# getterupper/PreWorld

Measured on AMD Instinct MI355X. Metric: samples/sec (6-cam frame -> 200x200x16 occ), higher is better.
Workload: dtype f32 as hi+lo f16 (3 MFMA per product block, f32 accumulate)

## Files before the change

### preworld_amd/csrc/pw_conv3d_common.h

```cpp
#ifndef PW_CONV3D_COMMON_H_
#define PW_CONV3D_COMMON_H_
#include "pw_common.h"

#include <stdlib.h>

typedef float f32x16 __attribute__((ext_vector_type(16)));

namespace {
constexpr int BD = 4, BH = 8, BW = 8;
constexpr int TD = BD + 2, TH = BH + 2, TW = BW + 2;
constexpr int TV = TD * TH * TW;
constexpr unsigned WPIECE = 1024u;
constexpr int KC = 32;
}

struct ConvArgs {
  const float* x;
  const float* wpk;
  const float* scale;
  const float* bias;
  const float* residual;
  float* y0;
  float* y1;
  int B, D, H, W, Cin;
// ... 111 lines not shown
  for (int mt = 0; mt < 2; ++mt) {
#pragma unroll
    for (int q = 0; q < 4; ++q) {
      const float av[4] = {aq[mt][q].x, aq[mt][q].y, aq[mt][q].z, aq[mt][q].w};
#pragma unroll
      for (int e = 0; e < 4; ++e) {
#pragma unroll
        for (int nt = 0; nt < NT; ++nt) {
          const float bv[4] = {b[nt][q].x, b[nt][q].y, b[nt][q].z, b[nt][q].w};
          acc[mt][nt] = __builtin_amdgcn_mfma_f32_32x32x2f32(av[e], bv[e], acc[mt][nt], 0, 0, 0);
        }
      }
    }
  }
}

template <int NT, int TAP>
__device__ __forceinline__ void tap_pair(const float* lds, const unsigned (&aaddr)[2][3][4],
                                         rsrc_t wr, unsigned wsoff, unsigned lane_off, unsigned wstride,
                                         float4 (&b0)[NT][4], float4 (&b1)[NT][4],
                                         f32x16 (&acc)[2][NT]) {
  if constexpr (TAP + 1 < 27) {
    load_b<NT>(wr, wsoff + (unsigned)(TAP + 1) * wstride, lane_off, b1);
    __builtin_amdgcn_sched_barrier(0);
    tap_mfma<NT, TAP>(lds, aaddr, b0, acc);
    __builtin_amdgcn_sched_barrier(0);
    load_b<NT>(wr, wsoff + (unsigned)(TAP + 2) * wstride, lane_off, b0);
    __builtin_amdgcn_sched_barrier(0);
    tap_mfma<NT, TAP + 1>(lds, aaddr, b1, acc);
    __builtin_amdgcn_sched_barrier(0);
    tap_pair<NT, TAP + 2>(lds, aaddr, wr, wsoff, lane_off, wstride, b0, b1, acc);
  } else {
    tap_mfma<NT, TAP>(lds, aaddr, b0, acc);
  }
}

__device__ __forceinline__ constexpr int acc_patch(int r, int h) {
  const int i = (r & 3) + 8 * (r >> 2) + 4 * h;
  const int g = i >> 2;
  const int set = (0x96 >> g) & 1;
  return set * 16 + (g >> 1) * 4 + (i & 3);
}

__device__ __forceinline__ int xcd_contiguous(int bid, int nblk) {
  const int x = bid & 7, idx = bid >> 3;
  const int q = nblk >> 3, r = nblk & 7;
  return x * q + min(x, r) + idx;
}

typedef __attribute__((address_space(3))) char* lds3_t;
constexpr unsigned PIPE_OOB = 0xfffffff0u;
constexpr int PIPE_BUF_BYTES = TV * KC * 4;
constexpr int PIPE_ROWS_PER_WAVE = TD * TH / 4;

struct PipeDma {
  unsigned voff[2][2];
  int b, d0, h0, wbase, ch;
  unsigned ldsbuf;
  bool live;
};

__device__ __forceinline__ void pipe_lane_offsets(const ConvArgs& a, int w0, int lane, unsigned (&voff)[2][2]) {
  const int shift = w0 == 0 ? 1 : 0;
  {
    const int ww = lane >> 3, slot = lane & 7;
    const bool wok = (unsigned)(w0 - 1 + ww) < (unsigned)a.W;
#pragma unroll
    for (int par = 0; par < 2; ++par) {
      const int f = ((ww >> 1) & 3) | (par << 2);
      voff[par][0] = wok ? (unsigned)((ww - shift) * a.Cin + (slot ^ f) * 4) * 4u : PIPE_OOB;
    }
  }
  {
    const int ww = 8 + (lane >> 5), dw = lane & 31, slot = dw >> 2;
    const bool wok = (unsigned)(w0 - 1 + ww) < (unsigned)a.W;
#pragma unroll
    for (int par = 0; par < 2; ++par) {
      const int f = ((ww >> 1) & 3) | (par << 2);
      voff[par][1] = wok ? (unsigned)((ww - shift) * a.Cin + (slot ^ f) * 4 + (dw & 3)) * 4u : PIPE_OOB;
    }
  }
}

template <int K>
__device__ __forceinline__ void pipe_dma_row(const ConvArgs& a, rsrc_t xr, lds3_t lds3, const PipeDma& dm,
                                             int wave) {
  const int row = wave + 4 * K;
  const int dd = row / TH, hh = row - dd * TH;
  const int gd = dm.d0 + dd - 1, gh = dm.h0 + hh - 1;
  const bool rok = dm.live && (unsigned)gd < (unsigned)a.D && (unsigned)gh < (unsigned)a.H;
  const unsigned soff = rok ? (unsigned)(((((dm.b * a.D + gd) * a.H + gh) * a.W + dm.wbase) * a.Cin + dm.ch * KC) * 4) : 0u;
  const unsigned v0 = rok ? ((hh & 1) ? dm.voff[1][0] : dm.voff[0][0]) : PIPE_OOB;
  const unsigned v1 = rok ? ((hh & 1) ? dm.voff[1][1] : dm.voff[0][1]) : PIPE_OOB;
  lds3_t dst = lds3 + (dm.ldsbuf + (unsigned)row * (TW * 128));
  __builtin_amdgcn_raw_ptr_buffer_load_lds(xr, dst, 16, v0, soff, 0, 0);
  __builtin_amdgcn_raw_ptr_buffer_load_lds(xr, dst + 1024, 4, v1, soff, 0, 0);
}


__device__ __forceinline__ void stage_halo_chunk_dma(const ConvArgs& a, rsrc_t xr, float* lds, int b, int d0,
                                                     int h0, int w0, int ch, int wave, int lane) {
  if (ch > 0) __syncthreads();
  PipeDma dm;
  pipe_lane_offsets(a, w0, lane, dm.voff);
  dm.b = b; dm.d0 = d0; dm.h0 = h0; dm.wbase = w0 > 0 ? w0 - 1 : 0; dm.ch = ch; dm.ldsbuf = 0; dm.live = true;
  const lds3_t lds3 = (lds3_t)lds;
  pipe_dma_row<0>(a, xr, lds3, dm, wave); pipe_dma_row<1>(a, xr, lds3, dm, wave); pipe_dma_row<2>(a, xr, lds3, dm, wave);
  pipe_dma_row<3>(a, xr, lds3, dm, wave); pipe_dma_row<4>(a, xr, lds3, dm, wave); pipe_dma_row<5>(a, xr, lds3, dm, wave);
  pipe_dma_row<6>(a, xr, lds3, dm, wave); pipe_dma_row<7>(a, xr, lds3, dm, wave); pipe_dma_row<8>(a, xr, lds3, dm, wave);
  pipe_dma_row<9>(a, xr, lds3, dm, wave); pipe_dma_row<10>(a, xr, lds3, dm, wave); pipe_dma_row<11>(a, xr, lds3, dm, wave);
  pipe_dma_row<12>(a, xr, lds3, dm, wave); pipe_dma_row<13>(a, xr, lds3, dm, wave); pipe_dma_row<14>(a, xr, lds3, dm, wave);
  __builtin_amdgcn_s_waitcnt(0);
  __syncthreads();
}


struct PipeArgs {
  unsigned m_ng, m_tw, m_th, m_td;
  int ngroups, n_items;
};


__device__ __forceinline__ int udiv_magic(int x, int d, unsigned magic) {
  return d == 1 ? x : (int)__umulhi((unsigned)x, magic);
}

struct PipeTile { int b, d0, h0, w0, ng; };

__device__ __forceinline__ PipeTile pipe_decode(const ConvArgs& a, const PipeArgs& p, int item) {
  PipeTile t;
  int tile = udiv_magic(item, p.ngroups, p.m_ng);
  t.ng = item - tile * p.ngroups;
  int q = udiv_magic(tile, a.tiles_w, p.m_tw);
  t.w0 = (tile - q * a.tiles_w) * BW; tile = q;
  q = udiv_magic(tile, a.tiles_h, p.m_th);
  t.h0 = (tile - q * a.tiles_h) * BH; tile = q;
  q = udiv_magic(tile, a.tiles_d, p.m_td);
  t.d0 = (tile - q * a.tiles_d) * BD;
  t.b = q;
  return t;
}


template <typename K>
static int set_lds_limit(K kernel, int bytes) {
  PW_CHECK_HIP(hipFuncSetAttribute(reinterpret_cast<const void*>(kernel),
                                   hipFuncAttributeMaxDynamicSharedMemorySize, bytes));
  return PW_OK;
}

static inline unsigned magic_of(int d) { return d <= 1 ? 0u : (unsigned)((1ull << 32) / (unsigned)d) + 1u; }

static inline int pw_num_cus() {
  static int n = 0;
  if (!n) {
    int dev = 0;
    hipDeviceProp_t pr;
    if (hipGetDevice(&dev) == hipSuccess && hipGetDeviceProperties(&pr, dev) == hipSuccess) n = pr.multiProcessorCount;
    if (n < 8) n = 256;
  }
  return n;
}

static inline bool use_pipe(long long n_items, int NT, int algo) {
  if (algo == 1 || algo == 4) return algo == 4 && n_items < (1ll << 20);
  return NT == 1 && n_items >= 512 && n_items < (1ll << 20);
}

int pw_launch_conv3d_gather(const ConvArgs& a, int NT, int ngroups, int ksize, int stride, int algo, int Cin,
                             long long n_out, hipStream_t st, bool f16 = false);
int pw_launch_conv3d_h2_s2(const ConvArgs& a, hipStream_t st);

#endif
```

### preworld_amd/csrc/pw_conv3d_h2.hip

```cpp
#include "pw_h2.h"

namespace {
constexpr int H2_SB_OFF = 2 * PIPE_BUF_BYTES;
constexpr int H2_MAX_COUT = 256;
constexpr int H2_LDS = H2_SB_OFF + 2 * H2_MAX_COUT * 4;
}

struct EpiTile { int b, d0, h0, w0, ng; unsigned bufoff; bool pending; };
struct EpiRegs {
  v4f x0, x1, s0, s1, b0, b1; float4 r0, r1; unsigned vbase, soff;
  float amax0, amax1;
  float amax_nt[2];
};

template <int NT>
__device__ __forceinline__ void epi_fold_amax(const ConvArgs& a, int ng, EpiRegs& r) {
#pragma unroll
  for (int nt = 0; nt < NT; ++nt) {
    const bool to_y0 = (ng * NT + nt) * 32 < a.cout0;
    r.amax0 = fmaxf(r.amax0, to_y0 ? r.amax_nt[nt] : 0.f);
    r.amax1 = fmaxf(r.amax1, to_y0 ? 0.f : r.amax_nt[nt]);
    r.amax_nt[nt] = 0.f;
  }
}

__device__ __forceinline__ unsigned epi_slot_off(int u) {
  const int row = (int)(((unsigned)u * 205u) >> 11);
  return (unsigned)(row * (4 * TW * 128) + (u - row * 10) * 128);
}

template <int NT>
__device__ __forceinline__ void h2_epi_park(const f32x16 (&acc)[2][NT], char* stg, int lane) {
  const int half = lane >> 5, pj = patch_of_row(lane & 31);
#pragma unroll
  for (int nt = 0; nt < NT; ++nt)
#pragma unroll
    for (int mt = 0; mt < 2; ++mt) {
      const int u = nt * 64 + mt * 32 + pj;
      char* dst = stg + epi_slot_off(u);
      const int sw = (u >> 1) & 7;
#pragma unroll
      for (int g = 0; g < 4; ++g) {
        v4f v;
#pragma unroll
        for (int e = 0; e < 4; ++e) v[e] = acc[mt][nt][4 * g + e];
        *reinterpret_cast<v4f*>(dst + (((2 * g + half) ^ sw) * 16)) = v;
      }
    }
}

template <int NT, int EPI, int P>
__device__ __forceinline__ void h2_epi_load(const ConvArgs& a, const EpiTile& t, const char* stg, const float* sb, int wave,
                                            int lane, EpiRegs& r) {
  constexpr int nt = P >> 2;
  const int n0 = (t.ng * NT + nt) * 32;
  const bool to_y0 = n0 < a.cout0;
  const int ld = to_y0 ? a.ld0 : a.ld1;
  const int col0 = to_y0 ? n0 : n0 - a.n1_start;
  const int od = t.d0 + wave;
  const int o = lane & 3;
  const int u = 16 * P + (lane >> 2), sv = u & 63;
  const int mt = sv >> 5, vr = (sv >> 3) & 3, vc = sv & 7;
  const bool ok = (int)t.pending & (int)(od < a.Do) & (int)((t.h0 + mt * 4 + vr) < a.Ho) & (int)((t.w0 + vc) < a.Wo);
  r.soff = (unsigned)(((((t.b * a.Do + od) * a.Ho + t.h0) * a.Wo + t.w0) * ld) * 4);
  const unsigned pos = (EPI == 3 ? (unsigned)(32 * o) : (unsigned)((4 * (o & 1) + 2 * (o >> 1)) * 16));
  const unsigned vin = (unsigned)(((mt * 4 + vr) * a.Wo + vc) * ld) * 4u + (unsigned)col0 * 4u + pos;
  r.vbase = ok ? vin : PIPE_OOB;
  const char* src = stg + epi_slot_off(u);
  const int sw = (u >> 1) & 7;
  r.x0 = *reinterpret_cast<const v4f*>(src + (((2 * o) ^ sw) * 16));
  r.x1 = *reinterpret_cast<const v4f*>(src + (((2 * o + 1) ^ sw) * 16));
  r.s0 = *reinterpret_cast<const v4f*>(sb + n0 + 8 * o);
  r.s1 = *reinterpret_cast<const v4f*>(sb + n0 + 8 * o + 4);
  r.b0 = *reinterpret_cast<const v4f*>(sb + H2_MAX_COUT + n0 + 8 * o);
  r.b1 = *reinterpret_cast<const v4f*>(sb + H2_MAX_COUT + n0 + 8 * o + 4);
  if constexpr (EPI == 2) {
    const unsigned out_vox = (unsigned)((size_t)a.B * a.Do * a.Ho * a.Wo);
    const rsrc_t rr = make_rsrc(a.residual, out_vox * (unsigned)ld * 4u);
    r.r0 = buf_load4(rr, r.vbase, r.soff);
    r.r1 = buf_load4(rr, r.vbase == PIPE_OOB ? PIPE_OOB : r.vbase + 16u, r.soff);
  }
}

template <int NT, int EPI, int P>
__device__ __forceinline__ void h2_epi_compute(const ConvArgs& a, const EpiTile& t, EpiRegs& r, float res_mul) {
  constexpr int nt = P >> 2;
  const int n0 = (t.ng * NT + nt) * 32;
  const bool to_y0 = n0 < a.cout0;
  float* dst = to_y0 ? a.y0 : a.y1;
  const int ld = to_y0 ? a.ld0 : a.ld1;
  const float lo_clamp = (to_y0 ? a.relu0 : a.relu1) ? 0.f : -3.402823466e38f;
  const unsigned out_vox = (unsigned)((size_t)a.B * a.Do * a.Ho * a.Wo);
  const rsrc_t yr = make_rsrc(dst, out_vox * (unsigned)ld * 4u);
  float v[8];
#pragma unroll
  for (int e = 0; e < 4; ++e) { v[e] = fmaf(r.x0[e], r.s0[e], r.b0[e]); v[4 + e] = fmaf(r.x1[e], r.s1[e], r.b1[e]); }
  if constexpr (EPI == 2) {
    const h8 rh = __builtin_bit_cast(h8, r.r0), rl = __builtin_bit_cast(h8, r.r1);
#pragma unroll
    for (int e = 0; e < 8; ++e) v[e] = fmaf((float)rh[e] + (float)rl[e], res_mul, v[e]);
  }
#pragma unroll
  for (int e = 0; e < 8; ++e) v[e] = fmaxf(v[e], lo_clamp);
  {
    float m = fabsf(v[0]);
#pragma unroll
    for (int e = 1; e < 8; ++e) m = fmaxf(m, fabsf(v[e]));
    r.amax_nt[nt] = fmaxf(r.amax_nt[nt], r.vbase == PIPE_OOB ? 0.f : m);
  }
  const unsigned second = r.vbase == PIPE_OOB ? PIPE_OOB : r.vbase + 16u;
  if constexpr (EPI == 3) {
    const float va[4] = {v[0], v[1], v[2], v[3]}, vb[4] = {v[4], v[5], v[6], v[7]};
    buf_store4(yr, r.vbase, r.soff, va);
    buf_store4(yr, second, r.soff, vb);
  } else {
    h8 oh, ol;
    h2_split8(v, oh, ol);
    const v4f wh = __builtin_bit_cast(v4f, oh), wl = __builtin_bit_cast(v4f, ol);
    const float va[4] = {wh[0], wh[1], wh[2], wh[3]}, vb[4] = {wl[0], wl[1], wl[2], wl[3]};
    buf_store4(yr, r.vbase, r.soff, va);
    buf_store4(yr, second, r.soff, vb);
  }
}

template <int NT, int EPI, int P>
__device__ __forceinline__ void h2_epi_rest(const ConvArgs& a, const EpiTile& t, const char* stg, const float* sb, int wave,
                                            int lane, EpiRegs& r, float res_mul) {
  if constexpr (P < 4 * NT) {
    h2_epi_load<NT, EPI, P>(a, t, stg, sb, wave, lane, r);
    h2_epi_compute<NT, EPI, P>(a, t, r, res_mul);
    h2_epi_rest<NT, EPI, P + 1>(a, t, stg, sb, wave, lane, r, res_mul);
  }
}

#ifndef PW_DMA_ROWS_PER_TAP_NT1
#define PW_DMA_ROWS_PER_TAP_NT1 3
#endif
#ifndef PW_DMA_ROWS_PER_TAP_NT2
#define PW_DMA_ROWS_PER_TAP_NT2 5
#endif
template <int NT, int TAP>
__device__ __forceinline__ constexpr int h2_dma_first_row() {
  constexpr int per = NT == 1 ? PW_DMA_ROWS_PER_TAP_NT1 : PW_DMA_ROWS_PER_TAP_NT2, t0 = 4 * NT + 2;
  return TAP < t0 ? PIPE_ROWS_PER_WAVE : (TAP - t0) * per;
}
template <int NT, int TAP>
__device__ __forceinline__ constexpr int h2_dma_row_count() {
  constexpr int per = NT == 1 ? PW_DMA_ROWS_PER_TAP_NT1 : PW_DMA_ROWS_PER_TAP_NT2;
  constexpr int k0 = h2_dma_first_row<NT, TAP>();
  return k0 >= PIPE_ROWS_PER_WAVE ? 0 : (k0 + per <= PIPE_ROWS_PER_WAVE ? per : PIPE_ROWS_PER_WAVE - k0);
}

template <int NT>
struct H2Ctx {
  lds3_t lds3;
  rsrc_t xr, wr;
  unsigned lane_off, wstride;
  unsigned wsoff, wsoff_next;
  bool has_next;
  PipeDma dm;
  unsigned dm_base, dm_pitch;
  int wave, lane;
  long long* tap_probe;
  EpiTile epi;
  const char* ldsg;
  float res_mul;
};

template <int TAP>
__device__ __forceinline__ void h2_read_a_tap(lds3_t lds3, const unsigned (&aaddr)[2][3][4], v4f (&aq)[2][4]) {
  constexpr int kd = TAP / 9, kh = (TAP / 3) % 3, kw = TAP % 3;
#pragma unroll
  for (int mt = 0; mt < 2; ++mt) {
    constexpr unsigned imm0 = (unsigned)(((kd * TH + kh) * TW) * 128);
    const unsigned imm = imm0 + (unsigned)(mt * 4 * TW * 128);
#pragma unroll
    for (int q = 0; q < 4; ++q)
      aq[mt][q] = *reinterpret_cast<const __attribute__((address_space(3))) v4f*>(lds3 + aaddr[kh & 1][kw][q] + imm);
  }
}

template <int NT, bool WR = false>
__device__ __forceinline__ void h2_load_b(rsrc_t wr, unsigned wsoff, unsigned lane_off, v4f (&b)[NT][4]) {
#pragma unroll
  for (int nt = 0; nt < NT; ++nt)
#pragma unroll
    for (int q = WR ? 1 : 0; q < 4; q += WR ? 2 : 1) {
      const auto v = __builtin_amdgcn_raw_buffer_load_b128(wr, lane_off + (unsigned)q * H2W_PIECE, wsoff + (unsigned)(nt * 4096), 0);
      v4f o;
      o[0] = __uint_as_float(v[0]); o[1] = __uint_as_float(v[1]); o[2] = __uint_as_float(v[2]); o[3] = __uint_as_float(v[3]);
      b[nt][q] = o;
    }
}

template <int NT, bool WR = false, int TAP = 0, int NW = 1>
__device__ __forceinline__ void h2_mfma(const v4f (&aq)[2][4], const v4f (&b)[NT][4], f32x16 (&acc)[2][NT], const v4f (&wres)[NW][2]) {
#pragma unroll
  for (int ks = 0; ks < 2; ++ks) {
#pragma unroll
    for (int prod = 0; prod < 3; ++prod) {
      const int pw = prod == 1 ? 1 : 0, px = prod == 2 ? 1 : 0;
#pragma unroll
      for (int mt = 0; mt < 2; ++mt)
#pragma unroll
        for (int nt = 0; nt < NT; ++nt) {
          v4f w = b[nt][2 * ks + pw];
          if constexpr (WR) { if (pw == 0) w = wres[TAP][ks]; }
          acc[mt][nt] = __builtin_amdgcn_mfma_f32_32x32x16_f16(__builtin_bit_cast(h8, w), __builtin_bit_cast(h8, aq[mt][2 * ks + px]),
                                                               acc[mt][nt], 0, 0, 0);
        }
    }
  }
}
template <int NT>
__device__ __forceinline__ void h2_mfma(const v4f (&aq)[2][4], const v4f (&b)[NT][4], f32x16 (&acc)[2][NT]) {
  const v4f none[1][2] = {};
  h2_mfma<NT, false, 0, 1>(aq, b, acc, none);
}

__device__ __forceinline__ constexpr int h2_share(int i, int slots, int n) { return ((i + 1) * n) / slots - (i * n) / slots; }

template <int I, int S, int NVM, int NDS, int NSA, int NVA>
__device__ __forceinline__ void h2_pipeline() {
  if constexpr (I < S) {
    __builtin_amdgcn_sched_group_barrier(0x008, 1, 0);
    if constexpr (h2_share(I, S, NDS) > 0) __builtin_amdgcn_sched_group_barrier(0x100, h2_share(I, S, NDS), 0);
    if constexpr (h2_share(I, S, NVM) > 0) __builtin_amdgcn_sched_group_barrier(0x020, h2_share(I, S, NVM), 0);
    if constexpr (h2_share(I, S, NSA) > 0) __builtin_amdgcn_sched_group_barrier(0x004, h2_share(I, S, NSA), 0);
    if constexpr (h2_share(I, S, NVA) > 0) __builtin_amdgcn_sched_group_barrier(0x002, h2_share(I, S, NVA), 0);
    h2_pipeline<I + 1, S, NVM, NDS, NSA, NVA>();
  }
}

struct H2DmaView { rsrc_t xr; lds3_t lds3; unsigned base, pitch; int wave; };
template <int K>
__device__ __forceinline__ void h2_dma_row(const ConvArgs& a, const PipeDma& dm, const H2DmaView& c) {
  constexpr int c1 = (4 * K) / TH, c2 = (4 * K) % TH;
  const int t = c2 + c.wave;
  const int carry = t >= TH ? 1 : 0;
  const int dd = c1 + carry, hh = t - TH * carry;
  const bool rok = (int)dm.live & (int)((unsigned)(dm.d0 - 1 + dd) < (unsigned)a.D) & (int)((unsigned)(dm.h0 - 1 + hh) < (unsigned)a.H);
  const unsigned soff = c.base + (unsigned)(dd * a.H + hh) * c.pitch;
#ifdef PW_X_DMAOOB
  const unsigned v0 = rok ? PIPE_OOB : PIPE_OOB - 16u, v1 = v0;
#else
  const unsigned v0 = rok ? ((hh & 1) ? dm.voff[1][0] : dm.voff[0][0]) : PIPE_OOB;
  const unsigned v1 = rok ? ((hh & 1) ? dm.voff[1][1] : dm.voff[0][1]) : PIPE_OOB;
#endif
  lds3_t dst = c.lds3 + (dm.ldsbuf + (unsigned)(c1 * TH + c2) * (TW * 128) + (unsigned)c.wave * (TW * 128));
  __builtin_amdgcn_raw_ptr_buffer_load_lds(c.xr, dst, 16, v0, soff, 0, 0);
  __builtin_amdgcn_raw_ptr_buffer_load_lds(c.xr, dst + 1024, 4, v1, soff, 0, 0);
}

template <int K0, int N>
__device__ __forceinline__ void h2_dma_rows(const ConvArgs& a, const PipeDma& dm, const H2DmaView& c) {
  if constexpr (N > 0) {
    h2_dma_row<K0>(a, dm, c);
    h2_dma_rows<K0 + 1, N - 1>(a, dm, c);
  }
}

template <int NT, int EPI, int TAP, bool WR = false, int NW = 1>
__device__ __forceinline__ void h2_step(const ConvArgs& a, const H2Ctx<NT>& c, const unsigned (&aaddr)[2][3][4],
                                        v4f (&ac)[2][4], v4f (&an)[2][4], v4f (&b0)[NT][4], v4f (&b1)[NT][4],
                                        v4f (&b2)[NT][4], f32x16 (&acc)[2][NT], EpiRegs& er, const v4f (&wres)[NW][2]) {
#ifdef PW_CONV_TAP_PROBE
  if (c.tap_probe) {
    if (c.lane == 0) c.tap_probe[c.wave * 27 + TAP] = __builtin_readcyclecounter();
  }
#endif
  __builtin_amdgcn_sched_barrier(0);
  constexpr int dma_k0 = h2_dma_first_row<NT, TAP>(), dma_n = h2_dma_row_count<NT, TAP>();
#ifdef PW_X_NOEPI
  constexpr bool epi_tap = false, epi_ld = false;
#else
  constexpr bool epi_tap = EPI > 0 && TAP >= 2 && TAP <= 4 * NT + 1;
  constexpr bool epi_ld = EPI > 0 && TAP >= 1 && TAP <= 4 * NT;
#endif
#ifdef PW_X_BSAME
  h2_load_b<NT, WR>(c.wr, c.wsoff, c.lane_off, b2);
#elif !defined(PW_X_NOB)
  if constexpr (TAP + 2 < 27) {
    h2_load_b<NT, WR>(c.wr, c.wsoff + (unsigned)(TAP + 2) * c.wstride, c.lane_off, b2);
  } else {
    h2_load_b<NT, WR>(c.wr, c.wsoff_next + (unsigned)(TAP + 2 - 27) * c.wstride, c.lane_off, b2);
  }
#endif
#ifndef PW_X_NODMA
  h2_dma_rows<dma_k0, dma_n>(a, c.dm, H2DmaView{c.xr, c.lds3, c.dm_base, c.dm_pitch, c.wave});
#endif
#ifndef PW_X_NOA
  if constexpr (TAP < 26) h2_read_a_tap<TAP + 1>(c.lds3, aaddr, an);
#endif
  if constexpr (epi_tap) h2_epi_compute<NT, EPI, TAP - 2>(a, c.epi, er, c.res_mul);
  if constexpr (epi_ld)
    h2_epi_load<NT, EPI, TAP - 1>(a, c.epi, c.ldsg + c.epi.bufoff + (unsigned)c.wave * (TW * 128),
                                  reinterpret_cast<const float*>(c.ldsg + H2_SB_OFF), c.wave, c.lane, er);
  h2_mfma<NT, WR, TAP, NW>(ac, b0, acc, wres);
  {
    constexpr int n_vm = (WR ? 2 : 4) * NT + 2 * dma_n + ((epi_ld && EPI == 2) ? 2 : 0);
    constexpr int n_ds = (TAP < 26 ? 8 : 0) + (epi_ld ? 6 : 0);
    constexpr int n_sa = 4 + 26 * dma_n + (epi_ld ? 12 : 0);
    constexpr int n_va = 5 * dma_n + (epi_tap ? (EPI == 2 ? 100 : 76) : 0) + (epi_ld ? 36 : 0);
    h2_pipeline<0, 12 * NT, n_vm, n_ds, n_sa, n_va>();
    if constexpr (epi_tap) __builtin_amdgcn_sched_group_barrier(0x040, 2, 0);
  }
  __builtin_amdgcn_sched_barrier(0);
  if constexpr (TAP < 26) h2_step<NT, EPI, TAP + 1, WR, NW>(a, c, aaddr, an, ac, b1, b2, b0, acc, er, wres);
}

template <int NT>
__device__ __forceinline__ void h2_epilogue(const ConvArgs& a, const f32x16 (&acc)[2][NT], const float* sb, char* stg,
                                            int b, int d0, int h0, int w0, int ng, int wave, int lane, float res_mul,
                                            float& amax0, float& amax1) {
  const int od = d0 + wave;
  const int half = lane >> 5, pj = patch_of_row(lane & 31);
  const unsigned out_vox = (unsigned)((size_t)a.B * a.Do * a.Ho * a.Wo);
  constexpr unsigned STG_ROW = 4 * TW * 128;
#pragma unroll
  for (int nt = 0; nt < NT; ++nt) {
    const int n0 = (ng * NT + nt) * 32;
    const bool to_y0 = n0 < a.cout0;
    float* dst = to_y0 ? a.y0 : a.y1;
    if (dst == nullptr) continue;
    const int stride = to_y0 ? a.cout0 : a.cout1;
    const int ld = to_y0 ? a.ld0 : a.ld1;
    const int col0 = to_y0 ? n0 : n0 - a.n1_start;
    if (col0 < 0 || col0 >= stride) continue;
    const int fmt = to_y0 ? a.fmt_y0 : a.fmt_y1;
    const float lo_clamp = (to_y0 ? a.relu0 : a.relu1) ? 0.f : -3.402823466e38f;
    const bool has_res = to_y0 && a.residual != nullptr;
    const rsrc_t yr = make_rsrc(dst, out_vox * (unsigned)ld * 4u);
    const rsrc_t rr = make_rsrc(has_res ? a.residual : dst, out_vox * (unsigned)ld * 4u);
#pragma unroll
    for (int g = 0; g < 4; ++g) {
      const v4f sc = *reinterpret_cast<const v4f*>(sb + n0 + 8 * g + 4 * half);
      const v4f bi = *reinterpret_cast<const v4f*>(sb + H2_MAX_COUT + n0 + 8 * g + 4 * half);
#pragma unroll
      for (int mt = 0; mt < 2; ++mt) {
        const int sv = mt * 32 + pj;
        v4f v;
#pragma unroll
        for (int e = 0; e < 4; ++e) v[e] = fmaf(acc[mt][nt][4 * g + e], sc[e], bi[e]);
        *reinterpret_cast<v4f*>(stg + (sv >> 3) * STG_ROW + (sv & 7) * 128 + (((2 * g + half) ^ ((sv >> 1) & 7)) * 16)) = v;
      }
    }
    const int o = lane & 3;
#pragma unroll
    for (int q = 0; q < 4; ++q) {
      const int sv = 16 * q + (lane >> 2);
      const int mt = sv >> 5, vr = (sv >> 3) & 3, vc = sv & 7;
      const bool ok = od < a.Do && (h0 + mt * 4 + vr) < a.Ho && (w0 + vc) < a.Wo;
      const unsigned soff = (unsigned)(((((b * a.Do + od) * a.Ho + h0) * a.Wo + w0) * ld) * 4);
      const unsigned vox = (unsigned)(((mt * 4 + vr) * a.Wo + vc) * ld) * 4u + (unsigned)col0 * 4u;
      const char* src = stg + (sv >> 3) * STG_ROW + (sv & 7) * 128;
      const int sw = (sv >> 1) & 7;
      const v4f lo4 = *reinterpret_cast<const v4f*>(src + (((2 * o) ^ sw) * 16));
      const v4f hi4 = *reinterpret_cast<const v4f*>(src + (((2 * o + 1) ^ sw) * 16));
      float v[8] = {lo4[0], lo4[1], lo4[2], lo4[3], hi4[0], hi4[1], hi4[2], hi4[3]};
      const unsigned pos = (fmt == 0 ? (unsigned)(32 * o) : (unsigned)((4 * (o & 1) + 2 * (o >> 1)) * 16));
      const unsigned rpos = (a.fmt_res == 0 ? (unsigned)(32 * o) : (unsigned)((4 * (o & 1) + 2 * (o >> 1)) * 16));
      if (has_res) {
        const unsigned base = ok ? vox + rpos : PIPE_OOB;
        const float4 r0 = buf_load4(rr, base, soff), r1 = buf_load4(rr, ok ? base + 16u : PIPE_OOB, soff);
        if (a.fmt_res == 0) {
          const float rv[8] = {r0.x, r0.y, r0.z, r0.w, r1.x, r1.y, r1.z, r1.w};
#pragma unroll
          for (int e = 0; e < 8; ++e) v[e] = fmaf(rv[e], res_mul, v[e]);
        } else {
          const h8 rh = __builtin_bit_cast(h8, r0), rl = __builtin_bit_cast(h8, r1);
#pragma unroll
          for (int e = 0; e < 8; ++e) v[e] = fmaf((float)rh[e] + (float)rl[e], res_mul, v[e]);
        }
      }
#pragma unroll
      for (int e = 0; e < 8; ++e) v[e] = fmaxf(v[e], lo_clamp);
      if (ok) {
        float m = fabsf(v[0]);
#pragma unroll
        for (int e = 1; e < 8; ++e) m = fmaxf(m, fabsf(v[e]));
        if (to_y0) amax0 = fmaxf(amax0, m); else amax1 = fmaxf(amax1, m);
      }
      const unsigned obase = ok ? vox + pos : PIPE_OOB;
      if (fmt == 0) {
        const float va[4] = {v[0], v[1], v[2], v[3]}, vb[4] = {v[4], v[5], v[6], v[7]};
        buf_store4(yr, obase, soff, va);
        buf_store4(yr, ok ? obase + 16u : PIPE_OOB, soff, vb);
      } else {
        h8 oh, ol;
        h2_split8(v, oh, ol);
        const v4f wh = __builtin_bit_cast(v4f, oh), wl = __builtin_bit_cast(v4f, ol);
        const float va[4] = {wh[0], wh[1], wh[2], wh[3]}, vb[4] = {wl[0], wl[1], wl[2], wl[3]};
        buf_store4(yr, obase, soff, va);
        buf_store4(yr, ok ? obase + 16u : PIPE_OOB, soff, vb);
      }
    }
  }
}

template <int NT, int EPI, bool WR = false>
__global__ void __launch_bounds__(256, 1) k_conv3d_h2(ConvArgs a, PipeArgs p) {
#ifdef PW_X_SKIP_SMALLCONV
  if ((long long)a.D * a.H * a.W <= 80000) return;
#endif
#ifdef PW_X_SKIP_BIGCONV
  if ((long long)a.D * a.H * a.W > 80000) return;
#endif
  extern __shared__ __attribute__((aligned(16))) float lds[];
  const int tid = threadIdx.x, lane = tid & 63;
  const int wave = uni(tid >> 6);
  const int half = lane >> 5, j = lane & 31;
  const int pj = patch_of_row(j), pr = pj >> 3, pc = pj & 7;
  const int ntiles_total = a.cout_total >> 5;
  const int nchunk = a.Cin / KC;

  const RngScale rs = rng_scales(a);

  const int nslots = (int)gridDim.x >> 3;
  const int per = (p.n_items + 7) >> 3;
  const int it_end = min(((int)blockIdx.x & 7) * per + per, p.n_items);
  int item = ((int)blockIdx.x & 7) * per + ((int)blockIdx.x >> 3);
  if (item >= it_end) return;

  unsigned aaddr0[2][3][4];
#pragma unroll
  for (int khp = 0; khp < 2; ++khp)
#pragma unroll
    for (int kw = 0; kw < 3; ++kw) {
      const int ww = pc + kw;
      const int f = ((ww >> 1) & 3) | (((pr + khp) & 1) << 2);
#pragma unroll
      for (int q = 0; q < 4; ++q)
        aaddr0[khp][kw][q] = (unsigned)((((wave * TH + pr) * TW + ww) * 8 + ((half * 4 + q) ^ f)) * 16);
    }

  H2Ctx<NT> c;
  c.lds3 = (lds3_t)lds;
  c.xr = make_rsrc(a.x, (unsigned)((size_t)a.B * a.D * a.H * a.W * a.Cin * 4));
  c.wr = make_rsrc(a.wpk, (unsigned)((size_t)nchunk * 27 * ntiles_total * 4096));
  c.lane_off = (unsigned)lane * 16u;
  c.wstride = (unsigned)ntiles_total * 4096u;
  c.wave = wave; c.lane = lane;
  c.ldsg = reinterpret_cast<const char*>(lds);
  c.epi.pending = false; c.epi.b = c.epi.d0 = c.epi.h0 = c.epi.w0 = c.epi.ng = 0; c.epi.bufoff = 0;

  constexpr int NW = WR ? 27 : 1;
  v4f wres[NW][2] = {};
  if constexpr (WR) {
#pragma unroll
    for (int tp = 0; tp < 27; ++tp)
#pragma unroll
      for (int ks = 0; ks < 2; ++ks) {
        const auto v = __builtin_amdgcn_raw_buffer_load_b128(c.wr, c.lane_off + (unsigned)(2 * ks) * H2W_PIECE, (unsigned)tp * c.wstride, 0);
        v4f o;
        o[0] = __uint_as_float(v[0]); o[1] = __uint_as_float(v[1]); o[2] = __uint_as_float(v[2]); o[3] = __uint_as_float(v[3]);
        wres[tp][ks] = o;
      }
  }
  PipeTile t = pipe_decode(a, p, item);
  int ch = 0;
  v4f a0[2][4], a1[2][4], b0[NT][4], b1[NT][4], b2[NT][4];
  EpiRegs er = {};
  f32x16 acc[2][NT];
#pragma unroll
  for (int mt = 0; mt < 2; ++mt)
#pragma unroll
    for (int nt = 0; nt < NT; ++nt)
#pragma unroll
      for (int r = 0; r < 16; ++r) acc[mt][nt][r] = 0.f;

  {
    PipeDma dm;
    pipe_lane_offsets(a, t.w0, lane, dm.voff);
    dm.b = t.b; dm.d0 = t.d0; dm.h0 = t.h0; dm.wbase = t.w0 > 0 ? t.w0 - 1 : 0; dm.ch = 0; dm.ldsbuf = 0;
    dm.live = true;
    h2_load_b<NT, WR>(c.wr, (unsigned)((t.ng * NT) * 4096), c.lane_off, b0);
    h2_load_b<NT, WR>(c.wr, (unsigned)((t.ng * NT) * 4096) + c.wstride, c.lane_off, b1);
    pipe_dma_row<0>(a, c.xr, c.lds3, dm, wave); pipe_dma_row<1>(a, c.xr, c.lds3, dm, wave);
    pipe_dma_row<2>(a, c.xr, c.lds3, dm, wave); pipe_dma_row<3>(a, c.xr, c.lds3, dm, wave);
    pipe_dma_row<4>(a, c.xr, c.lds3, dm, wave); pipe_dma_row<5>(a, c.xr, c.lds3, dm, wave);
    pipe_dma_row<6>(a, c.xr, c.lds3, dm, wave); pipe_dma_row<7>(a, c.xr, c.lds3, dm, wave);
    pipe_dma_row<8>(a, c.xr, c.lds3, dm, wave); pipe_dma_row<9>(a, c.xr, c.lds3, dm, wave);
    pipe_dma_row<10>(a, c.xr, c.lds3, dm, wave); pipe_dma_row<11>(a, c.xr, c.lds3, dm, wave);
    pipe_dma_row<12>(a, c.xr, c.lds3, dm, wave); pipe_dma_row<13>(a, c.xr, c.lds3, dm, wave);
    pipe_dma_row<14>(a, c.xr, c.lds3, dm, wave);
    float* sb = lds + H2_SB_OFF / 4;
    for (int n = tid; n < a.cout_total; n += 256) {
      const bool to_y0 = n < a.cout0;
      sb[n] = (a.scale ? a.scale[n] : 1.f) * (to_y0 ? rs.s0 : rs.s1);
      sb[H2_MAX_COUT + n] = (a.bias ? a.bias[n] : 0.f) * (to_y0 ? rs.b0 : rs.b1);
    }
    c.res_mul = rs.res;
    __builtin_amdgcn_s_waitcnt(0);
    __syncthreads();
  }

  for (int stage = 0;; ++stage) {
    const unsigned bufoff = (stage & 1) ? (unsigned)PIPE_BUF_BYTES : 0u;
    unsigned aaddr[2][3][4];
#pragma unroll
    for (int khp = 0; khp < 2; ++khp)
#pragma unroll
      for (int kw = 0; kw < 3; ++kw)
#pragma unroll
        for (int q = 0; q < 4; ++q) {
          aaddr[khp][kw][q] = aaddr0[khp][kw][q] + bufoff;
          asm volatile("" : "+v"(aaddr[khp][kw][q]));
        }
    long long ts0 = 0, ts1 = 0, ts2 = 0;
    if (a.probe) ts0 = __builtin_readcyclecounter();
    h2_read_a_tap<0>(c.lds3, aaddr, a0);

    PipeTile tn = t;
    int chn = ch + 1, itemn = item;
    if (chn == nchunk) { chn = 0; itemn = item + nslots; }
    c.has_next = itemn < it_end;
    if (c.has_next && chn == 0) tn = pipe_decode(a, p, itemn);
    if (!c.has_next) chn = 0;
    c.wsoff = (unsigned)((ch * 27 * ntiles_total + t.ng * NT) * 4096);
    c.wsoff_next = (unsigned)((chn * 27 * ntiles_total + tn.ng * NT) * 4096);
    pipe_lane_offsets(a, tn.w0, lane, c.dm.voff);
    c.dm.b = tn.b; c.dm.d0 = tn.d0; c.dm.h0 = tn.h0; c.dm.wbase = tn.w0 > 0 ? tn.w0 - 1 : 0;
    c.dm.ch = chn; c.dm.ldsbuf = (unsigned)PIPE_BUF_BYTES - bufoff; c.dm.live = c.has_next;
    c.dm_pitch = (unsigned)(a.W * a.Cin) * 4u;
    c.dm_base = (unsigned)(((((tn.b * a.D + tn.d0 - 1) * a.H + tn.h0 - 1) * a.W + c.dm.wbase) * a.Cin + chn * KC) * 4);

    c.tap_probe = (a.probe && blockIdx.x == 17 && stage == 3) ? a.probe + 256 * 8 * 16 * 4 : nullptr;
    h2_step<NT, EPI, 0, WR, NW>(a, c, aaddr, a0, a1, b0, b1, b2, acc, er, wres);
    if (a.probe) ts1 = __builtin_readcyclecounter();

    __builtin_amdgcn_s_waitcnt(0);
    __syncthreads();
    if (a.probe) ts2 = __builtin_readcyclecounter();

    if constexpr (EPI > 0) { if (c.epi.pending) epi_fold_amax<NT>(a, c.epi.ng, er); }
    c.epi.pending = false;
    if (ch == nchunk - 1) {
      char* stg = reinterpret_cast<char*>(lds) + bufoff + (unsigned)wave * (TW * 128);
      if constexpr (EPI == 0) {
        h2_epilogue<NT>(a, acc, lds + H2_SB_OFF / 4, stg, t.b, t.d0, t.h0, t.w0, t.ng, wave, lane, rs.res, er.amax0, er.amax1);
      } else {
        h2_epi_park<NT>(acc, stg, lane);
        c.epi.b = t.b; c.epi.d0 = t.d0; c.epi.h0 = t.h0; c.epi.w0 = t.w0; c.epi.ng = t.ng; c.epi.bufoff = bufoff;
        c.epi.pending = true;
      }
#pragma unroll
      for (int mt = 0; mt < 2; ++mt)
#pragma unroll
        for (int nt = 0; nt < NT; ++nt)
#pragma unroll
          for (int r = 0; r < 16; ++r) acc[mt][nt][r] = 0.f;
    }
    if (a.probe && lane == 0 && stage < 16) {
      long long* pp = a.probe + (((size_t)blockIdx.x * 8 + wave) * 16 + stage) * 4;
      pp[0] = ts0; pp[1] = ts1; pp[2] = ts2; pp[3] = __builtin_readcyclecounter();
    }
    if (!c.has_next) break;
    t = tn; ch = chn; item = itemn;
  }
  if constexpr (EPI > 0) {
    if (c.epi.pending)
      h2_epi_rest<NT, EPI, 0>(a, c.epi, reinterpret_cast<const char*>(lds) + c.epi.bufoff + (unsigned)wave * (TW * 128),
                              lds + H2_SB_OFF / 4, wave, lane, er, rs.res);
    if (c.epi.pending) epi_fold_amax<NT>(a, c.epi.ng, er);
  }
  if (a.fmt_y0) rng_note(a.y0_rng, __float_as_uint(er.amax0), rs.e0);
  if (a.fmt_y1 && a.y1) rng_note(a.y1_rng, __float_as_uint(er.amax1), rs.e1);
}


__global__ void __launch_bounds__(256) k_rng_fold(int* tab, int* compact) {
  int* r = tab + (size_t)blockIdx.x * PW_RNG_ROW;
  __shared__ unsigned sm[4];
  unsigned m = 0u;
  for (int k = threadIdx.x; k < PW_RNG_WORDS; k += 256) {
    m = max(m, (unsigned)r[PW_RNG_SCRATCH + k]);
    r[PW_RNG_SCRATCH + k] = 0;
  }
#pragma unroll
  for (int off = 32; off; off >>= 1) m = max(m, (unsigned)__shfl_xor((int)m, off));
  if ((threadIdx.x & 63) == 0) sm[threadIdx.x >> 6] = m;
  __syncthreads();
  if (threadIdx.x == 0) {
    m = max(max(sm[0], sm[1]), max(sm[2], sm[3]));
    m = max(m, (unsigned)r[1]);
    r[1] = (int)m;
    if (compact) { compact[2 * blockIdx.x] = r[0]; compact[2 * blockIdx.x + 1] = (int)m; }
  }
}
__global__ void k_rng_clear(int* rng) { rng[1] = 0; }
__global__ void k_rng_pick(int* rng) { rng[0] = rng_ideal_exp((unsigned)rng[1]); rng[1] = 0; }

PW_API int pw_rng_fold(int32_t* tab, int n_slots, int32_t* compact, void* stream) {
  PW_CHECK_ARG(tab && n_slots > 0, "pw_rng_fold: bad arguments");
  hipLaunchKernelGGL(k_rng_fold, dim3((unsigned)n_slots), dim3(256), 0, pw_stream(stream), tab, compact);
  PW_CHECK_LAUNCH();
  return PW_OK;
}

__global__ void __launch_bounds__(256) k_rng_audit(const int* __restrict__ compact, int n_slots, int* sticky) {
  __shared__ int bad;
  if (threadIdx.x == 0) bad = 0;
  __syncthreads();
  for (int i = threadIdx.x; i < n_slots; i += 256) {
    const unsigned bits = (unsigned)compact[2 * i + 1];
    if (bits == 0u) continue;
    const float stored = __builtin_ldexpf(__uint_as_float(bits), -compact[2 * i]);
    if (!(stored >= 64.f && stored <= H2_MAX)) atomicAdd(&bad, 1);
  }
  __syncthreads();
  if (threadIdx.x == 0) {
// ... 193 lines not shown
```

Measured before the change: 396.9.

## Share A fragments across adjacent output rows in NT=1 conv path

For NT=1, each wave's two M-tiles now cover adjacent output rows instead of rows four apart. The row-shifted A fragment for kh can then be reused as the other tile's fragment for the next kh, which removes part of the LDS reads per tap. To keep bank-conflict-free access, the LDS XOR swizzle parity switches from the row to row>>1 in both the DMA and read addressing, and the epilogue and parking positions are remapped to match. The cost is a six-slot fragment register file in place of two double-buffered pairs, which can raise VGPR pressure.

```diff
diff --git a/preworld_amd/csrc/pw_conv3d_common.h b/preworld_amd/csrc/pw_conv3d_common.h
--- a/preworld_amd/csrc/pw_conv3d_common.h
+++ b/preworld_amd/csrc/pw_conv3d_common.h
@@ -217,7 +217,7 @@
   }
 }
 
-template <int K>
+template <int K, int HSH = 0>
 __device__ __forceinline__ void pipe_dma_row(const ConvArgs& a, rsrc_t xr, lds3_t lds3, const PipeDma& dm,
                                              int wave) {
   const int row = wave + 4 * K;
@@ -225,8 +225,8 @@
   const int gd = dm.d0 + dd - 1, gh = dm.h0 + hh - 1;
   const bool rok = dm.live && (unsigned)gd < (unsigned)a.D && (unsigned)gh < (unsigned)a.H;
   const unsigned soff = rok ? (unsigned)(((((dm.b * a.D + gd) * a.H + gh) * a.W + dm.wbase) * a.Cin + dm.ch * KC) * 4) : 0u;
-  const unsigned v0 = rok ? ((hh & 1) ? dm.voff[1][0] : dm.voff[0][0]) : PIPE_OOB;
-  const unsigned v1 = rok ? ((hh & 1) ? dm.voff[1][1] : dm.voff[0][1]) : PIPE_OOB;
+  const unsigned v0 = rok ? (((hh >> HSH) & 1) ? dm.voff[1][0] : dm.voff[0][0]) : PIPE_OOB;
+  const unsigned v1 = rok ? (((hh >> HSH) & 1) ? dm.voff[1][1] : dm.voff[0][1]) : PIPE_OOB;
   lds3_t dst = lds3 + (dm.ldsbuf + (unsigned)row * (TW * 128));
   __builtin_amdgcn_raw_ptr_buffer_load_lds(xr, dst, 16, v0, soff, 0, 0);
   __builtin_amdgcn_raw_ptr_buffer_load_lds(xr, dst + 1024, 4, v1, soff, 0, 0);
diff --git a/preworld_amd/csrc/pw_conv3d_h2.hip b/preworld_amd/csrc/pw_conv3d_h2.hip
--- a/preworld_amd/csrc/pw_conv3d_h2.hip
+++ b/preworld_amd/csrc/pw_conv3d_h2.hip
@@ -5,6 +5,24 @@
 constexpr int H2_MAX_COUT = 256;
 constexpr int H2_LDS = H2_SB_OFF + 2 * H2_MAX_COUT * 4;
 }
+
+#ifndef PW_X_ROWSHARE
+#define PW_X_ROWSHARE 1
+#endif
+template <int NT>
+__device__ __forceinline__ constexpr bool h2_rowshare() { return PW_X_ROWSHARE == 2 || (PW_X_ROWSHARE == 1 && NT == 1); }
+template <int NT>
+__device__ __forceinline__ int h2_base_row(int pr) { return h2_rowshare<NT>() ? 2 * pr : pr; }
+template <int NT>
+__device__ __forceinline__ int h2_plane_pos(int pj, int mt) {
+  return (h2_base_row<NT>(pj >> 3) + (h2_rowshare<NT>() ? mt : 4 * mt)) * 8 + (pj & 7);
+}
+template <int NT, int TAP, int MT>
+__device__ __forceinline__ constexpr int h2_a_slot() {
+  return h2_rowshare<NT>() ? (TAP % 3) * 2 + (((TAP / 3) % 3 + MT) & 1) : (TAP & 1) * 2 + MT;
+}
+template <int NT, int TAP, int MT>
+__device__ __forceinline__ constexpr bool h2_a_load() { return !h2_rowshare<NT>() || MT == 1 || (TAP / 3) % 3 == 0; }
 
 struct EpiTile { int b, d0, h0, w0, ng; unsigned bufoff; bool pending; };
 struct EpiRegs {
@@ -36,7 +54,7 @@
   for (int nt = 0; nt < NT; ++nt)
 #pragma unroll
     for (int mt = 0; mt < 2; ++mt) {
-      const int u = nt * 64 + mt * 32 + pj;
+      const int u = nt * 64 + h2_plane_pos<NT>(pj, mt);
       char* dst = stg + epi_slot_off(u);
       const int sw = (u >> 1) & 7;
 #pragma unroll
@@ -167,18 +185,25 @@
   float res_mul;
 };
 
-template <int TAP>
-__device__ __forceinline__ void h2_read_a_tap(lds3_t lds3, const unsigned (&aaddr)[2][3][4], v4f (&aq)[2][4]) {
-  constexpr int kd = TAP / 9, kh = (TAP / 3) % 3, kw = TAP % 3;
-#pragma unroll
-  for (int mt = 0; mt < 2; ++mt) {
-    constexpr unsigned imm0 = (unsigned)(((kd * TH + kh) * TW) * 128);
-    const unsigned imm = imm0 + (unsigned)(mt * 4 * TW * 128);
+template <int NT, int TAP, int MT>
+__device__ __forceinline__ void h2_read_a_mt(lds3_t lds3, const unsigned (&aaddr)[2][3][4], v4f (&fr)[6][4]) {
+  if constexpr (h2_a_load<NT, TAP, MT>()) {
+    constexpr int kd = TAP / 9, kh = (TAP / 3) % 3, kw = TAP % 3;
+    constexpr int row = kh + (h2_rowshare<NT>() ? MT : 4 * MT);
+    constexpr unsigned imm = (unsigned)(((kd * TH + row) * TW) * 128);
 #pragma unroll
     for (int q = 0; q < 4; ++q)
-      aq[mt][q] = *reinterpret_cast<const __attribute__((address_space(3))) v4f*>(lds3 + aaddr[kh & 1][kw][q] + imm);
-  }
-}
+      fr[h2_a_slot<NT, TAP, MT>()][q] =
+          *reinterpret_cast<const __attribute__((address_space(3))) v4f*>(lds3 + aaddr[(row >> (h2_rowshare<NT>() ? 1 : 0)) & 1][kw][q] + imm);
+  }
+}
+template <int NT, int TAP>
+__device__ __forceinline__ void h2_read_a_tap(lds3_t lds3, const unsigned (&aaddr)[2][3][4], v4f (&fr)[6][4]) {
+  h2_read_a_mt<NT, TAP, 0>(lds3, aaddr, fr);
+  h2_read_a_mt<NT, TAP, 1>(lds3, aaddr, fr);
+}
+template <int NT, int TAP>
+__device__ __forceinline__ constexpr int h2_a_reads() { return 4 * ((int)h2_a_load<NT, TAP, 0>() + (int)h2_a_load<NT, TAP, 1>()); }
 
 template <int NT, bool WR = false>
 __device__ __forceinline__ void h2_load_b(rsrc_t wr, unsigned wsoff, unsigned lane_off, v4f (&b)[NT][4]) {
@@ -194,7 +219,8 @@
 }
 
 template <int NT, bool WR = false, int TAP = 0, int NW = 1>
-__device__ __forceinline__ void h2_mfma(const v4f (&aq)[2][4], const v4f (&b)[NT][4], f32x16 (&acc)[2][NT], const v4f (&wres)[NW][2]) {
+__device__ __forceinline__ void h2_mfma(const v4f (&fr)[6][4], const v4f (&b)[NT][4], f32x16 (&acc)[2][NT], const v4f (&wres)[NW][2]) {
+  constexpr int slot[2] = {h2_a_slot<NT, TAP, 0>(), h2_a_slot<NT, TAP, 1>()};
 #pragma unroll
   for (int ks = 0; ks < 2; ++ks) {
 #pragma unroll
@@ -206,16 +232,11 @@
         for (int nt = 0; nt < NT; ++nt) {
           v4f w = b[nt][2 * ks + pw];
           if constexpr (WR) { if (pw == 0) w = wres[TAP][ks]; }
-          acc[mt][nt] = __builtin_amdgcn_mfma_f32_32x32x16_f16(__builtin_bit_cast(h8, w), __builtin_bit_cast(h8, aq[mt][2 * ks + px]),
+          acc[mt][nt] = __builtin_amdgcn_mfma_f32_32x32x16_f16(__builtin_bit_cast(h8, w), __builtin_bit_cast(h8, fr[slot[mt]][2 * ks + px]),
                                                                acc[mt][nt], 0, 0, 0);
         }
     }
   }
-}
-template <int NT>
-__device__ __forceinline__ void h2_mfma(const v4f (&aq)[2][4], const v4f (&b)[NT][4], f32x16 (&acc)[2][NT]) {
-  const v4f none[1][2] = {};
-  h2_mfma<NT, false, 0, 1>(aq, b, acc, none);
 }
 
 __device__ __forceinline__ constexpr int h2_share(int i, int slots, int n) { return ((i + 1) * n) / slots - (i * n) / slots; }
@@ -233,7 +254,7 @@
 }
 
 struct H2DmaView { rsrc_t xr; lds3_t lds3; unsigned base, pitch; int wave; };
-template <int K>
+template <int K, int HSH>
 __device__ __forceinline__ void h2_dma_row(const ConvArgs& a, const PipeDma& dm, const H2DmaView& c) {
   constexpr int c1 = (4 * K) / TH, c2 = (4 * K) % TH;
   const int t = c2 + c.wave;
@@ -244,25 +265,25 @@
 #ifdef PW_X_DMAOOB
   const unsigned v0 = rok ? PIPE_OOB : PIPE_OOB - 16u, v1 = v0;
 #else
-  const unsigned v0 = rok ? ((hh & 1) ? dm.voff[1][0] : dm.voff[0][0]) : PIPE_OOB;
-  const unsigned v1 = rok ? ((hh & 1) ? dm.voff[1][1] : dm.voff[0][1]) : PIPE_OOB;
+  const unsigned v0 = rok ? (((hh >> HSH) & 1) ? dm.voff[1][0] : dm.voff[0][0]) : PIPE_OOB;
+  const unsigned v1 = rok ? (((hh >> HSH) & 1) ? dm.voff[1][1] : dm.voff[0][1]) : PIPE_OOB;
 #endif
   lds3_t dst = c.lds3 + (dm.ldsbuf + (unsigned)(c1 * TH + c2) * (TW * 128) + (unsigned)c.wave * (TW * 128));
   __builtin_amdgcn_raw_ptr_buffer_load_lds(c.xr, dst, 16, v0, soff, 0, 0);
   __builtin_amdgcn_raw_ptr_buffer_load_lds(c.xr, dst + 1024, 4, v1, soff, 0, 0);
 }
 
-template <int K0, int N>
+template <int K0, int N, int HSH>
 __device__ __forceinline__ void h2_dma_rows(const ConvArgs& a, const PipeDma& dm, const H2DmaView& c) {
   if constexpr (N > 0) {
-    h2_dma_row<K0>(a, dm, c);
-    h2_dma_rows<K0 + 1, N - 1>(a, dm, c);
+    h2_dma_row<K0, HSH>(a, dm, c);
+    h2_dma_rows<K0 + 1, N - 1, HSH>(a, dm, c);
   }
 }
 
 template <int NT, int EPI, int TAP, bool WR = false, int NW = 1>
 __device__ __forceinline__ void h2_step(const ConvArgs& a, const H2Ctx<NT>& c, const unsigned (&aaddr)[2][3][4],
-                                        v4f (&ac)[2][4], v4f (&an)[2][4], v4f (&b0)[NT][4], v4f (&b1)[NT][4],
+                                        v4f (&fr)[6][4], v4f (&b0)[NT][4], v4f (&b1)[NT][4],
                                         v4f (&b2)[NT][4], f32x16 (&acc)[2][NT], EpiRegs& er, const v4f (&wres)[NW][2]) {
 #ifdef PW_CONV_TAP_PROBE
   if (c.tap_probe) {
@@ -287,26 +308,26 @@
   }
 #endif
 #ifndef PW_X_NODMA
-  h2_dma_rows<dma_k0, dma_n>(a, c.dm, H2DmaView{c.xr, c.lds3, c.dm_base, c.dm_pitch, c.wave});
+  h2_dma_rows<dma_k0, dma_n, h2_rowshare<NT>() ? 1 : 0>(a, c.dm, H2DmaView{c.xr, c.lds3, c.dm_base, c.dm_pitch, c.wave});
 #endif
 #ifndef PW_X_NOA
-  if constexpr (TAP < 26) h2_read_a_tap<TAP + 1>(c.lds3, aaddr, an);
+  if constexpr (TAP < 26) h2_read_a_tap<NT, TAP + 1>(c.lds3, aaddr, fr);
 #endif
   if constexpr (epi_tap) h2_epi_compute<NT, EPI, TAP - 2>(a, c.epi, er, c.res_mul);
   if constexpr (epi_ld)
     h2_epi_load<NT, EPI, TAP - 1>(a, c.epi, c.ldsg + c.epi.bufoff + (unsigned)c.wave * (TW * 128),
                                   reinterpret_cast<const float*>(c.ldsg + H2_SB_OFF), c.wave, c.lane, er);
-  h2_mfma<NT, WR, TAP, NW>(ac, b0, acc, wres);
+  h2_mfma<NT, WR, TAP, NW>(fr, b0, acc, wres);
   {
     constexpr int n_vm = (WR ? 2 : 4) * NT + 2 * dma_n + ((epi_ld && EPI == 2) ? 2 : 0);
-    constexpr int n_ds = (TAP < 26 ? 8 : 0) + (epi_ld ? 6 : 0);
+    constexpr int n_ds = (TAP < 26 ? h2_a_reads<NT, TAP + 1 < 27 ? TAP + 1 : 0>() : 0) + (epi_ld ? 6 : 0);
     constexpr int n_sa = 4 + 26 * dma_n + (epi_ld ? 12 : 0);
     constexpr int n_va = 5 * dma_n + (epi_tap ? (EPI == 2 ? 100 : 76) : 0) + (epi_ld ? 36 : 0);
     h2_pipeline<0, 12 * NT, n_vm, n_ds, n_sa, n_va>();
     if constexpr (epi_tap) __builtin_amdgcn_sched_group_barrier(0x040, 2, 0);
   }
   __builtin_amdgcn_sched_barrier(0);
-  if constexpr (TAP < 26) h2_step<NT, EPI, TAP + 1, WR, NW>(a, c, aaddr, an, ac, b1, b2, b0, acc, er, wres);
+  if constexpr (TAP < 26) h2_step<NT, EPI, TAP + 1, WR, NW>(a, c, aaddr, fr, b1, b2, b0, acc, er, wres);
 }
 
 template <int NT>
@@ -338,7 +359,7 @@
       const v4f bi = *reinterpret_cast<const v4f*>(sb + H2_MAX_COUT + n0 + 8 * g + 4 * half);
 #pragma unroll
       for (int mt = 0; mt < 2; ++mt) {
-        const int sv = mt * 32 + pj;
+        const int sv = h2_plane_pos<NT>(pj, mt);
         v4f v;
 #pragma unroll
         for (int e = 0; e < 4; ++e) v[e] = fmaf(acc[mt][nt][4 * g + e], sc[e], bi[e]);
@@ -422,16 +443,18 @@
   int item = ((int)blockIdx.x & 7) * per + ((int)blockIdx.x >> 3);
   if (item >= it_end) return;
 
+  constexpr int HSH = h2_rowshare<NT>() ? 1 : 0;
   unsigned aaddr0[2][3][4];
+  const int row0 = h2_base_row<NT>(pr);
 #pragma unroll
   for (int khp = 0; khp < 2; ++khp)
 #pragma unroll
     for (int kw = 0; kw < 3; ++kw) {
       const int ww = pc + kw;
-      const int f = ((ww >> 1) & 3) | (((pr + khp) & 1) << 2);
+      const int f = ((ww >> 1) & 3) | ((((row0 >> HSH) + khp) & 1) << 2);
 #pragma unroll
       for (int q = 0; q < 4; ++q)
-        aaddr0[khp][kw][q] = (unsigned)((((wave * TH + pr) * TW + ww) * 8 + ((half * 4 + q) ^ f)) * 16);
+        aaddr0[khp][kw][q] = (unsigned)((((wave * TH + row0) * TW + ww) * 8 + ((half * 4 + q) ^ f)) * 16);
     }
 
   H2Ctx<NT> c;
@@ -459,7 +482,7 @@
   }
   PipeTile t = pipe_decode(a, p, item);
   int ch = 0;
-  v4f a0[2][4], a1[2][4], b0[NT][4], b1[NT][4], b2[NT][4];
+  v4f fr[6][4], b0[NT][4], b1[NT][4], b2[NT][4];
   EpiRegs er = {};
   f32x16 acc[2][NT];
 #pragma unroll
@@ -476,14 +499,14 @@
     dm.live = true;
     h2_load_b<NT, WR>(c.wr, (unsigned)((t.ng * NT) * 4096), c.lane_off, b0);
     h2_load_b<NT, WR>(c.wr, (unsigned)((t.ng * NT) * 4096) + c.wstride, c.lane_off, b1);
-    pipe_dma_row<0>(a, c.xr, c.lds3, dm, wave); pipe_dma_row<1>(a, c.xr, c.lds3, dm, wave);
-    pipe_dma_row<2>(a, c.xr, c.lds3, dm, wave); pipe_dma_row<3>(a, c.xr, c.lds3, dm, wave);
-    pipe_dma_row<4>(a, c.xr, c.lds3, dm, wave); pipe_dma_row<5>(a, c.xr, c.lds3, dm, wave);
-    pipe_dma_row<6>(a, c.xr, c.lds3, dm, wave); pipe_dma_row<7>(a, c.xr, c.lds3, dm, wave);
-    pipe_dma_row<8>(a, c.xr, c.lds3, dm, wave); pipe_dma_row<9>(a, c.xr, c.lds3, dm, wave);
-    pipe_dma_row<10>(a, c.xr, c.lds3, dm, wave); pipe_dma_row<11>(a, c.xr, c.lds3, dm, wave);
-    pipe_dma_row<12>(a, c.xr, c.lds3, dm, wave); pipe_dma_row<13>(a, c.xr, c.lds3, dm, wave);
-    pipe_dma_row<14>(a, c.xr, c.lds3, dm, wave);
+    pipe_dma_row<0, HSH>(a, c.xr, c.lds3, dm, wave); pipe_dma_row<1, HSH>(a, c.xr, c.lds3, dm, wave);
+    pipe_dma_row<2, HSH>(a, c.xr, c.lds3, dm, wave); pipe_dma_row<3, HSH>(a, c.xr, c.lds3, dm, wave);
+    pipe_dma_row<4, HSH>(a, c.xr, c.lds3, dm, wave); pipe_dma_row<5, HSH>(a, c.xr, c.lds3, dm, wave);
+    pipe_dma_row<6, HSH>(a, c.xr, c.lds3, dm, wave); pipe_dma_row<7, HSH>(a, c.xr, c.lds3, dm, wave);
+    pipe_dma_row<8, HSH>(a, c.xr, c.lds3, dm, wave); pipe_dma_row<9, HSH>(a, c.xr, c.lds3, dm, wave);
+    pipe_dma_row<10, HSH>(a, c.xr, c.lds3, dm, wave); pipe_dma_row<11, HSH>(a, c.xr, c.lds3, dm, wave);
+    pipe_dma_row<12, HSH>(a, c.xr, c.lds3, dm, wave); pipe_dma_row<13, HSH>(a, c.xr, c.lds3, dm, wave);
+    pipe_dma_row<14, HSH>(a, c.xr, c.lds3, dm, wave);
     float* sb = lds + H2_SB_OFF / 4;
     for (int n = tid; n < a.cout_total; n += 256) {
       const bool to_y0 = n < a.cout0;
@@ -509,7 +532,7 @@
         }
     long long ts0 = 0, ts1 = 0, ts2 = 0;
     if (a.probe) ts0 = __builtin_readcyclecounter();
-    h2_read_a_tap<0>(c.lds3, aaddr, a0);
+    h2_read_a_tap<NT, 0>(c.lds3, aaddr, fr);
 
     PipeTile tn = t;
     int chn = ch + 1, itemn = item;
@@ -526,7 +549,7 @@
     c.dm_base = (unsigned)(((((tn.b * a.D + tn.d0 - 1) * a.H + tn.h0 - 1) * a.W + c.dm.wbase) * a.Cin + chn * KC) * 4);
 
     c.tap_probe = (a.probe && blockIdx.x == 17 && stage == 3) ? a.probe + 256 * 8 * 16 * 4 : nullptr;
-    h2_step<NT, EPI, 0, WR, NW>(a, c, aaddr, a0, a1, b0, b1, b2, acc, er, wres);
+    h2_step<NT, EPI, 0, WR, NW>(a, c, aaddr, fr, b0, b1, b2, acc, er, wres);
     if (a.probe) ts1 = __builtin_readcyclecounter();
 
     __builtin_amdgcn_s_waitcnt(0);
```

New measurement: 398.3, median of 4. No clear change (+0.3%).
